# eth-cscs/COSTA

Hardware: AMD Instinct MI355X
Metric: GB/s device-resident tile pack+transpose+unpack (fp64), % HBM peak (higher is better)
Workload: dtype f64; 1 GPU; pxtran fp64 16384x16384, 256x256 blocks, op T, alpha=1 beta=0, 1x1 grid (BASELINE configs[1]); op=T, parallelism=1 rank(s), one per GPU, RCCL send/recv exchange, m=16384, n=16384, block=256, grid=1x1

## Files before the change

### costa_amd/__init__.py

```python
from __future__ import annotations

import ctypes as C
import os
import struct
from dataclasses import dataclass
from typing import Iterable, Sequence

import numpy as np

__all__ = [
    "CostaError", "lib", "FLOAT", "DOUBLE", "CFLOAT", "CDOUBLE", "INT32", "HALF", "BFLOAT16",
    "FP8_E4M3", "FP8_E5M2", "FP4_E2M1", "FP6_E2M3", "FP6_E3M2", "dtype_code", "element_code",
    "np_dtype", "Layout", "block_cyclic_layout", "custom_layout", "Comm", "transform",
    "transform_batch", "transform_async", "transform_batch_async", "synchronize", "transformer", "copy_and_transform", "execute_tiles", "execute_tiles_mixed",
    "convert_subtile", "TileOp", "TriOp", "TRI_OP_DTYPE", "transform_tri", "transform_tri_async",
    "execute_tiles_tri", "plan_export_tri", "tri_cut", "tri_subtile", "tri_phase_ms",
    "plan_export", "set_profiling", "get_stats", "release_caches", "TILE_OP_DTYPE",
    "ScaledOp", "SCALED_OP_DTYPE", "SCALED_F_ROWS", "transform_scaled", "execute_tiles_scaled",
    "plan_export_scaled", "scaled_subtile", "scaled_items", "mx_subtile", "block_subtile",
    "transform_amax", "layout_amax", "execute_tiles_amax", "amax_items",
    "MxScales", "MX_ROWS", "MX_COLS", "MX_FLOOR", "MX_CEIL", "mx_scales", "transform_mx",
    "execute_tiles_mx", "mx_items", "sr_bits", "mx_check_ops", "mx_check_scales",
    "BlockScales", "BLOCK_EXACT", "BLOCK_POW2", "block_scales", "transform_block_scaled",
    "execute_tiles_block_scaled", "block_items", "block_check_ops", "block_check_scales",
]

FLOAT, DOUBLE, CFLOAT, CDOUBLE, INT32 = 0, 1, 2, 3, 4
HALF, BFLOAT16 = 5, 6
_NP = {FLOAT: np.float32, DOUBLE: np.float64, CFLOAT: np.complex64,
       CDOUBLE: np.complex128, INT32: np.int32, HALF: np.float16, BFLOAT16: np.uint16}
_TORCH = {"torch.float32": FLOAT, "torch.float64": DOUBLE, "torch.complex64": CFLOAT,
          "torch.complex128": CDOUBLE, "torch.int32": INT32, "torch.float16": HALF,
# ... 252 lines not shown
        "costa_hip_mx_check_scales": (i, [C.POINTER(MxScales), i64, i64]),
        "costa_hip_plan_export_scaled": (i, [vp, vp, c, vp, vp, i, i, C.POINTER(ScaledPlanInfo), vp, vp,
                                             vp, vp, vp, vp, vp, vp]),
        "costa_hip_plan_export": (i, [i, C.POINTER(vp), C.POINTER(vp), C.c_char_p, vp, vp, i, i,
                                      C.POINTER(PlanInfo), vp, vp, vp, vp, vp, vp, vp, vp]),
        "costa_hip_set_profiling": (i, [i]),
        "costa_hip_get_stats": (i, [C.POINTER(FullStats), i]),
        "costa_hip_release_caches": (i, []),
        "costa_hip_set_host_staging": (i, [i]),
        "costa_hip_set_planner": (i, [i]),
        "costa_hip_plan_export_device": (i, [i, i, C.POINTER(vp), C.POINTER(vp), C.c_char_p, vp, vp,
                                             i, i, C.POINTER(PlanInfo), vp, vp, vp, vp, vp, vp, vp,
                                             vp]),
        "costa_hip_set_list_builder": (i, [i]),
        "costa_hip_work_export": (i, [i, vp, i64, i, i, vp, i64, vp, i64, C.POINTER(i64)]),
    }
    for name, (res, args) in sig.items():
        try:
            f = getattr(L, name)
        except AttributeError:
            if os.environ.get("COSTA_LIB"):
                continue
            raise
        f.restype = res
        f.argtypes = args
    _lib = L
    return L


def _check(rc: int):
# ... 843 lines not shown
    code = element_code(dtype)
    ops = np.ascontiguousarray(ops, dtype=TILE_OP_DTYPE)
    k = {"local": 0, "pack": 1, "unpack": 2}[kind]
    dev = -1 if device is None else int(device)
    meta = (C.c_int64 * 12)()
    L = lib()
    _check(L.costa_hip_work_export(code, ops.ctypes.data, ops.size, k, dev, None, 0, None, 0, meta))
    o = np.zeros(meta[8], TILE_OP_DTYPE)
    w = np.zeros(meta[9], np.uint64)
    _check(L.costa_hip_work_export(code, ops.ctypes.data, ops.size, k, dev, o.ctypes.data, o.size,
                                   w.ctypes.data, w.size, meta))
    m = dict(zip(_WORK_META, list(meta)))
    return WorkLists(o, w, m, bool(m["on_gpu"]))


def set_host_staging(mode: int):
    _check(lib().costa_hip_set_host_staging(int(mode)))


def rccl_version() -> int:
    v = C.c_int(0)
    _check(lib().costa_hip_rccl_version(C.byref(v)))
    return v.value
```

### costa_amd/csrc/capi.cpp

```cpp
#include "engine.hpp"

#include <hip/hip_runtime.h>

#include <costa/transform.hpp>

#include <algorithm>
#include <cctype>
#include <complex>
#include <cstring>
#include <new>

struct costa_layout_s {
    costa::engine::elayout e;
    std::vector<int> base_owners;
};
struct costa_comm_s {
    costa::engine::comm* c = nullptr;
};

namespace {
thread_local std::string g_last_error;

template <typename F>
int guarded(F&& f) {
// ... 984 lines not shown
        const bool on_gpu = costa::engine::work_export(
            costa_dtype_t(dtype), in, costa::engine::list_kind(kind), device, o, w, ws);
        const int64_t m[12] = {ws.n_large, ws.n_medium, ws.n_skew, ws.n_cblock, ws.cblock_lds, ws.cb_map,
                               ws.tiny_first, ws.n_tiny, int64_t(o.size()), int64_t(w.size()), on_gpu,
                               int64_t(ws.tr_shape) | int64_t(ws.sq) << 1 | int64_t(ws.full) << 2 |
                                   int64_t(ws.med_full) << 3 | int64_t(ws.med_sq) << 4 |
                                   int64_t(ws.skew_wide) << 5};
        std::memcpy(meta, m, sizeof(m));
        if (ordered && cap_ordered >= int64_t(o.size()) && !o.empty())
            std::memcpy(ordered, o.data(), o.size() * sizeof(o[0]));
        if (work && cap_work >= int64_t(w.size()) && !w.empty()) std::memcpy(work, w.data(), w.size() * sizeof(w[0]));
    };
    return device >= 0 ? gpu_guarded(body) : guarded(body);
}

int costa_hip_set_profiling(int on) {
    costa::engine::set_profiling(on != 0);
    return COSTA_OK;
}

int costa_hip_get_stats(costa_stats_t* out, int reset) {
    return guarded([&] {
        if (!out) throw costa::engine::error(COSTA_ERR_ARG, "null argument");
        costa::engine::resolve_pending();
        *out = costa::engine::stats();
        if (reset) costa::engine::stats() = costa_stats_t{};
    });
}

int costa_hip_set_host_staging(int mode) {
// ... 152 lines not shown
```

### costa_amd/csrc/engine.cpp

```cpp
#include <exception>
#include <thread>
#include "engine.hpp"
#include "strip_work.hpp"

#include <hip/hip_runtime.h>
#include <rccl/rccl.h>

#include <algorithm>
#include <numeric>
#include <chrono>
#include <cmath>
#include <cstdio>
#include <cstdlib>
#include <cstring>
#include <deque>
#include <list>
#include <map>
#include <mutex>
#include <unordered_map>

namespace costa {
namespace engine {

#define HIP_CHECK(x)                                                                   \
// ... 964 lines not shown
                out.push_back(head);
            }
            if (h < op.nf) {
                costa_tile_op_t body = part;
                body.src += uint64_t(h * E);
                body.dst += uint64_t(h * E);
                body.nf = int32_t(op.nf - h);
                body.flags = (op.flags & ~vec_bits) | vec_flags(body.src, body.lds, body.dst, body.ldd, E) | keep_vs;
                out.push_back(body);
            }
        }
    }
    return true;
}

work_split build_work(costa_dtype_t dtype, const std::vector<costa_tile_op_t>& ops_in,
                      std::vector<costa_tile_op_t>& ordered, std::vector<uint64_t>& work,
                      list_kind kind, device_section* dev, bool dst_order) {
    const bool pack_list = kind == list_pack, local = kind == list_local;
    static const int mis_env = [] {
        const char* s = tuning_env("COSTA_MISALIGNED_VEC");
        return s ? std::atoi(s) : -1;
    }();
    const int mis = mis_env >= 0 ? mis_env : dtype_size(dtype) == 4 ? 2 : 0;
    const wave_knobs& kn0 = knobs();
    static const bool trace = std::getenv("COSTA_PLAN_TRACE") != nullptr;
    const auto bw0 = std::chrono::steady_clock::now();
    double bw_t[4] = {0, 0, 0, 0};
    double sub_t[3] = {0, 0, 0};
    auto lap = [&](int k) {
        if (!trace) return;
        const double t = std::chrono::duration<double, std::milli>(std::chrono::steady_clock::now() - bw0).count();
        bw_t[k] = t;
// ... 136 lines not shown
        if (cls[li] == 1) --n_med;
        if (groups_on && op.ns <= op.ldd && op.ldd <= group_budget) {
            cls[li] = 2;
            continue;
        }
        cls[li] = 4;
    }
    mark(2);
    std::vector<uint32_t> shaped[3];
    std::vector<costa_tile_op_t> skew_ops;
    for (size_t li = 0; li < ops.size(); ++li) {
        const int c = cls[li] == 1 && n_med < kMinMediumOps ? 2 : cls[li];
        if (c < 2) shaped[c].push_back(uint32_t(li));
        else if (c == 2) wave_ops.push_back(&ops[li]);
        else if (c == 4) skew_ops.push_back(ops[li]);
    }
    merge_adjacent(skew_ops, E);
    for (size_t i = 0; i < skew_ops.size(); ++i) shaped[2].push_back(uint32_t(i));
    bool skew_wide = false;
    for (const auto& op : skew_ops)
        skew_wide = skew_wide || (E == 4 && (op.src % 16 != 0 || (uint64_t(op.lds) * uint64_t(E)) % 16 != 0));
    const int64_t skew_group = kn.skew_xcd >= 0 ? kn.skew_xcd : skew_wide ? kSkewWideGroup : 0;
    int64_t n_work[3] = {0, 0, 0};
    for (int c = 0; c < 3; ++c) {
        const int bf = c == 2 ? (skew_wide ? sh.bf_kw : sh.bf_k) : c ? (med_sq ? sh.bf_s : sh.bf_m) : sq ? sh.bf_q : sh.bf;
        const int bs = c == 2 ? (skew_wide ? sh.bs_kw : sh.bs_k) : c ? (med_sq ? sh.bs_s : sh.bs_m) : sq ? sh.bs_q : sh.bs;
        const std::vector<uint32_t>& sel = shaped[c];
        const std::vector<costa_tile_op_t>& src_ops = c == 2 ? skew_ops : ops;
        std::vector<uint32_t> sperm(sel.size());
        for (size_t i = 0; i < sel.size(); ++i) sperm[i] = uint32_t(i);
// ... 139 lines not shown
        std::sort(key.begin(), key.end());
        for (size_t i = 0; i < nw; ++i) perm[i] = key[i].second;
    } else {
        for (size_t i = 0; i < nw; ++i) perm[i] = uint32_t(i);
    }
    if (kn.xcd_bands && mode == 2 && top > 0 && nw > 1) xcd_bands(wave_ops, E, kn.xcd_bands, local, perm);
    lap(2);
    std::vector<wave_grid> grid(nw);
    std::vector<size_t> at_piece(nw + 1, 0);
    host_parallel(nw, [&](size_t b, size_t e) {
        for (size_t i = b; i < e; ++i) grid[i] = wave_pieces(*wave_ops[perm[i]], E, local);
    });
    for (size_t i = 0; i < nw; ++i)
        at_piece[i + 1] = at_piece[i] + size_t(grid[i].nfc * grid[i].nsc);
    work_split w;
    w.tr_shape = tr_shape;
    w.sq = sq;
    w.full = tr_shape && !sq && !shaped[0].empty();
    for (const uint32_t li : shaped[0]) {
        const costa_tile_op_t& op = ops[li];
        w.full = w.full && (op.flags & vec_both) == vec_both && op.nf % sh.bf == 0 && op.ns % sh.bs == 0;
    }
    w.med_sq = med_sq && !shaped[1].empty();
    w.med_full = !shaped[1].empty() && n_work[1] > 0 && !w.med_sq;
    for (const uint32_t li : shaped[1])
        w.med_full = w.med_full && ops[li].nf % sh.bf_m == 0 && ops[li].ns % sh.bs_m == 0;
    w.n_large = n_work[0];
    w.n_medium = n_work[1];
    w.n_skew = n_work[2];
    w.skew_wide = skew_wide && n_work[2] > 0;
// ... 167 lines not shown

void set_layout_hash(elayout& L) { layout_hashes(L, L.hash, L.hash2); }

namespace {

struct dev_list {
    dbuf ops, work;
    template <typename Op>
    const Op* list() const { return static_cast<const Op*>(ops.p); }
    const uint64_t* items() const { return static_cast<const uint64_t*>(work.p); }
};

struct phase_lists {
    dev_list tiles;
    work_split split;
    strip_list convert;
    bool transposes = false, reads_c = false;
    dev_list tri;
    strip_list tri_items;
    dev_list scaled;
    strip_list scaled_items;
    dbuf block_work;
    strip_list block_items;
    bool empty() const {
        return !split.n_items() && !convert.n_items && !tri_items.n_items && !scaled_items.n_items;
    }
};

struct cached_plan {
    std::unique_ptr<plan> p;
// ... 137 lines not shown
    sec.device = device;
    sec.stream = dc.main;
    sec.force = true;
    w = build_work(dtype, ops, ordered, work, kind, &sec);
    if (!sec.n_ordered) return false;
    std::vector<costa_tile_op_t> o(sec.n_ordered);
    std::vector<uint64_t> k(sec.n_work);
    HIP_CHECK(hipMemcpyAsync(o.data(), sec.d_ordered, o.size() * sizeof(o[0]), hipMemcpyDeviceToHost, dc.main));
    HIP_CHECK(hipMemcpyAsync(k.data(), sec.d_work, k.size() * sizeof(k[0]), hipMemcpyDeviceToHost, dc.main));
    HIP_CHECK(hipStreamSynchronize(dc.main));
    ordered.insert(ordered.begin() + std::ptrdiff_t(sec.at_ordered), o.begin(), o.end());
    work.insert(work.begin() + std::ptrdiff_t(sec.at_work), k.begin(), k.end());
    return true;
}

namespace {
std::unique_ptr<plan> plan_jobs(const std::vector<job>& jobs, comm* c, hipStream_t s) {
    const int lb = c->size == 1 && c->nccl ? loopback_exchange() : 0;
    const int mode = planner_mode();
    size_t blocks = 0;
    for (const job& j : jobs) blocks += j.A->blocks.size() + j.C->blocks.size();
    const size_t need = g_device_planner_warm ? kDevicePlanBlocks : kColdDevicePlanBlocks;
    if (!any_packed(jobs) && (mode == 2 || (mode == 1 && blocks >= need))) {
        if (auto p = make_plan_device(jobs, c->rank, c->size, lb, c->device, s)) {
            g_stats.device_plans++;
            g_device_planner_warm = true;
            return p;
        }
    }
    return make_plan(jobs, c->rank, c->size, lb);
// ... 38 lines not shown
        sec.stream = s;
    }
};

void build_phase(const plan& p, list_kind kind, bool masked, const std::vector<costa_tile_op_t>& tiles,
                 const std::vector<costa_tri_op_t>& tri, const std::vector<costa_scaled_op_t>& scaled,
                 host_lists& h) {
    phase_lists& ph = *h.into;
    const dtype_pair t = phase_dtypes(p, kind);
    ph.transposes = kind != list_pack && any_transpose(tiles);
    ph.reads_c = kind != list_pack && any_axpby(tiles);
    switch (phase_tiles(p, kind)) {
    case tiles_on::converting:
        ph.convert = build_convert_work(t.src, t.dst, tiles, 0, 0, h.tiles, h.tiles_work);
        break;
    case tiles_on::tile_kernel:
        ph.split = build_work(t.dst, tiles, h.tiles, h.tiles_work, kind, kind == list_pack ? nullptr : &h.sec,
                              kind == list_local && masked);
        break;
    case tiles_on::none:
        break;
    }
    if (!tri.empty()) ph.tri_items = build_tri_work(t.dst, tri, 0, 0, h.tri, h.tri_work);
    if (scaled.empty()) return;
    static const bool local_by_dst = [] {
        const char* e = tuning_env("COSTA_SCALED_ORDER");
        return !e || std::atoi(e) != 0;
    }();
    const bool by_dst = kind == list_local && local_by_dst;
    ph.scaled_items = build_scaled_work(t.src, t.dst, scaled, 0, 0, h.scaled, h.scaled_work, by_dst);
    if (block_pair(p.src_dtype, p.dtype) && dtype_is_fp8(p.dtype)) {
        std::vector<costa_scaled_op_t> same;
        ph.block_items = build_block_work(t.src, t.dst, scaled, 0, 0, same, h.block_work, by_dst);
    }
}

void upload_phase(const host_lists& h, hipStream_t s) {
    phase_lists& ph = *h.into;
    upload_list(ph.tiles.ops, h.tiles, h.sec.d_ordered, h.sec.at_ordered, h.sec.n_ordered, s);
    upload_list(ph.tiles.work, h.tiles_work, h.sec.d_work, h.sec.at_work, h.sec.n_work, s);
    if (ph.tri_items.n_items) {
        ph.tri.ops.upload(h.tri, s);
        ph.tri.work.upload(h.tri_work, s);
    }
    if (ph.scaled_items.n_items) {
        ph.scaled.ops.upload(h.scaled, s);
        ph.scaled.work.upload(h.scaled_work, s);
    }
    if (ph.block_items.n_items) ph.block_work.upload(h.block_work, s);
}

template <typename Op>
std::vector<std::vector<Op>> by_round(const std::vector<Op>& ops, const std::vector<int>& round, int R) {
    std::vector<std::vector<Op>> out(static_cast<size_t>(R));
    for (size_t i = 0; i < ops.size(); ++i) out[size_t(round[i])].push_back(ops[i]);
    return out;
}

std::vector<host_lists> build_lists(cached_plan& cp, comm* c, hipStream_t s, bool masked) {
    const plan& p = *cp.p;
    if (p.packed() && (!p.local_ops.empty() || !p.unpack_ops.empty()))
        throw error(COSTA_ERR_INTERNAL, "costa: an FP4 / FP6 plan with ordinary LOCAL / UNPACK ops");
    const int R = c->exchanges() ? exchange_rounds() : 1;
    std::vector<int> pr, ur, tr, sr;
// ... 197 lines not shown
    if (masked || device_only(jobs)) {
        costa_dtype_t a, b;
        check_jobs(jobs, c->size, a, b);
    }
    auto cp = std::make_unique<cached_plan>();
    cp->device = c->device;
    staging st;
    if (stage_host_layouts(jobs, c, dc, masked, *cp, st)) return cp;
    const double t_resid = now_ms() - t0;
    cp->p = plan_jobs(st.jobs, c, dc.main);
    const double t_plan = now_ms() - t0 - t_resid;
    g_stats.plan_ms += t_plan;
    if (cp->staged) staged_copies(*cp, st, masked);
    const std::vector<host_lists> lists = build_lists(*cp, c, dc.main, masked);
    const double t_work = now_ms() - t0 - t_resid - t_plan;
    for (const host_lists& h : lists) upload_phase(h, dc.main);
    HIP_CHECK(hipStreamSynchronize(dc.main));
    if (trace)
        std::fprintf(stderr,
                     "[costa plan] %zu local / %zu pack / %zu unpack ops: residency %.2f ms, "
                     "planning %.2f, work lists %.2f, upload %.2f, total %.2f\n",
                     cp->p->local_ops.size(), cp->p->pack_ops.size(), cp->p->unpack_ops.size(), t_resid, t_plan,
                     t_work, now_ms() - t0 - t_resid - t_plan - t_work, now_ms() - t0);
    return cp;
}

cached_plan* get_plan(const std::vector<job>& jobs, comm* c, device_ctx& dc) {
    std::vector<uint64_t> key = plan_key(jobs, c);
    hasher h;
    for (uint64_t w : key) h.mix(w);
    for (auto it = g_plans.begin(); it != g_plans.end(); ++it) {
        if (it->h == h.h && it->key == key) {
// ... 28 lines not shown

void release_caches() {
    std::lock_guard<std::recursive_mutex> lk(g_mutex);
    g_plans.clear();
    release_host_rings();
    ctx_map().clear();
}

namespace {
enum phase { PH_LOCAL, PH_PACK, PH_EXCHANGE, PH_UNPACK, PH_H2D, PH_D2H, PH_TRI_LOCAL, PH_TRI_UNPACK };
double g_tri_ms = 0;
int64_t g_scaled_items = 0;
int64_t g_amax_items = 0;
int64_t g_mx_items = 0;
int64_t g_blk_items = 0;

struct phase_timer {
    device_ctx& dc;
    bool on;
    int ph = 0;
    hipEvent_t a = nullptr;
    hipStream_t s = nullptr;
    phase_timer(device_ctx& d, bool prof) : dc(d), on(prof) {}
    void start(int p, hipStream_t st) {
        if (!on) return;
        ph = p;
        s = st;
        a = dc.take_event();
        HIP_CHECK(hipEventRecord(a, s));
    }
// ... 35 lines not shown
        hipEvent_t e;
        HIP_CHECK(hipEventCreate(&e));
        return e;
    }
    hipEvent_t e = free_events.back();
    free_events.pop_back();
    return e;
}

void resolve_pending() {
    std::lock_guard<std::recursive_mutex> lk(g_mutex);
    for (auto& kv : ctx_map()) {
        HIP_CHECK(hipSetDevice(kv.first));
        kv.second->resolve();
    }
}

double tri_phase_ms(bool reset) {
    resolve_pending();
    std::lock_guard<std::recursive_mutex> lk(g_mutex);
    const double v = g_tri_ms;
    if (reset) g_tri_ms = 0;
    return v;
}

void synchronize(comm* c) {
    std::lock_guard<std::recursive_mutex> lk(g_mutex);
    if (!c) throw error(COSTA_ERR_ARG, "costa: null communicator");
    device_ctx& dc = ctx(c->device);
    HIP_CHECK(hipStreamSynchronize(dc.main));
// ... 183 lines not shown
    const int id = kind == list_local ? PH_LOCAL : kind == list_pack ? PH_PACK : PH_UNPACK;
    const void* scal = cp.d_scal.p;
    auto launch = [&](int phase, auto&& run) {
        if (after) HIP_CHECK(hipStreamWaitEvent(s, after, 0));
        tm.start(phase, s);
        run();
        tm.stop();
    };
    if (ph.convert.n_items)
        launch(id, [&] {
            launch_convert(t.src, t.dst, ph.tiles.list<costa_tile_op_t>(), ph.tiles.items(), ph.convert, src_base,
                           dst_base, scal, s);
        });
    if (ph.split.n_items())
        launch(id, [&] {
            launch_tiles(t.dst,
                         make_launch(ph.split, ph.tiles.ops.p, ph.tiles.work.p, src_base, dst_base, scal,
                                     ph.transposes, ph.reads_c),
                         s);
        });
    if (ph.tri_items.n_items)
        launch(kind == list_local ? PH_TRI_LOCAL : PH_TRI_UNPACK, [&] {
            launch_tri(t.dst, ph.tri.list<costa_tri_op_t>(), ph.tri.items(), ph.tri_items, src_base, dst_base, scal, s);
        });
    if (ph.scaled_items.n_items)
        launch(id, [&] {
            const costa_scaled_op_t* ops = ph.scaled.list<costa_scaled_op_t>();
            switch (sv.scheme) {
            case scale_scheme::block:
                launch_block(t.src, t.dst, ops,
                             sv.quantises() ? static_cast<const uint64_t*>(ph.block_work.p) : ph.scaled.items(),
                             sv.quantises() ? ph.block_items : ph.scaled_items, src_base, dst_base, scal,
                             sv.blk.a_scales, sv.blk.c_scales, sv.blk.pow2, s);
                break;
// ... 731 lines not shown
```

### costa_amd/csrc/engine.hpp

```cpp
#pragma once

#include <costa/layout.hpp>
#include <costa_hip.h>

#include <array>
#include <cstdint>
#include <functional>
#include <memory>
#include <string>
#include <vector>

#include "tile_op.hpp"

namespace costa {
namespace engine {

size_t dtype_size(costa_dtype_t t);
esize elem_size(costa_dtype_t t);
bool dtype_is_complex(costa_dtype_t t);
bool dtype_is_half(costa_dtype_t t);
costa_dtype_t compute_dtype(costa_dtype_t src, costa_dtype_t dst);
bool half_pair(costa_dtype_t src, costa_dtype_t dst);
bool dtype_is_fp8(costa_dtype_t t);
bool fp8_pair(costa_dtype_t src, costa_dtype_t dst);
// ... 289 lines not shown
    const char* src_base;
    char* dst_base;
    const void* scalars;
    bool any_transpose;
    bool any_axpby;
    bool tr_shape;
    bool sq;
    bool full;
    bool med_full;
    bool med_sq;
    bool skew_wide = false;
};
bool any_transpose(const std::vector<costa_tile_op_t>& ops);
bool any_axpby(const std::vector<costa_tile_op_t>& ops);
void launch_tiles(costa_dtype_t dtype, const launch_args& a, void* stream );
bool pieces_in_group_launch(int64_t n_cblock, int64_t n_tiny);
constexpr int64_t kPanelBytes = int64_t(128) << 10;
constexpr int kCblockThreads = 256;
constexpr int kCblockChunks = 4;
inline int64_t cblock_max_elems(int64_t E) { return int64_t(kCblockThreads) * kCblockChunks * (16 / E); }
constexpr int64_t kCblockXcdChunk = 16;
constexpr int64_t cblock_xcd_order(int64_t b, int64_t nb, int64_t ch = kCblockXcdChunk) {
    return b / (8 * ch) * (8 * ch) + 8 * ch <= nb ? b / (8 * ch) * (8 * ch) + (b % 8) * ch + (b / 8) % ch : b;
}
constexpr int64_t xcd_slice_order(int64_t b, int64_t nb) {
    return (b % 8) < nb % 8 ? (b % 8) * (nb / 8 + 1) + b / 8
                            : (nb % 8) * (nb / 8 + 1) + ((b % 8) - nb % 8) * (nb / 8) + b / 8;
}
enum cblock_map { cb_round_robin = 0, cb_xcd_chunks = 1, cb_xcd_bands = 2 };
struct shape_dims {
// ... 17 lines not shown
    bool skew_wide = false;
    int64_t n_items() const { return n_large + n_medium + n_skew + n_cblock + n_tiny; }
};
enum list_kind { list_local, list_pack, list_unpack };
struct device_section {
    int device = -1;
    void* stream = nullptr;
    bool force = false;
    std::shared_ptr<void> mem;
    costa_tile_op_t* d_ordered = nullptr;
    uint64_t* d_work = nullptr;
    size_t at_ordered = 0, n_ordered = 0, at_work = 0, n_work = 0;
};
work_split build_work(costa_dtype_t dtype, const std::vector<costa_tile_op_t>& ops,
                      std::vector<costa_tile_op_t>& ordered, std::vector<uint64_t>& work,
                      list_kind kind = list_local, device_section* dev = nullptr, bool dst_order = false);
constexpr size_t kDeviceGroupsMin = 16384;
int list_builder_mode();
void set_list_builder_mode(int mode);
int64_t cblock_groups_device(int64_t E, int64_t budget, uint32_t vec_bits, int bands_env,
                             const std::vector<costa_tile_op_t>& ops, const std::vector<uint32_t>& wave,
                             size_t base_at, device_section& sec, std::vector<char>& taken,
                             int64_t& lds, int& map);
bool work_export(costa_dtype_t dtype, const std::vector<costa_tile_op_t>& ops, list_kind kind,
                 int device, std::vector<costa_tile_op_t>& ordered, std::vector<uint64_t>& work,
                 work_split& w);
launch_args make_launch(const work_split& w, const void* d_ordered, const void* d_work,
                        const char* src_base, char* dst_base, const void* d_scalars, bool transpose,
                        bool axpby);

struct host_pipeline;
// ... 31 lines not shown
```

### costa_amd/csrc/tile_kernels.hip

```cpp
#include <hip/hip_runtime.h>

#include <algorithm>
#include <cstdlib>
#include <type_traits>

#include "engine.hpp"
#include "tile_device.hpp"

#pragma clang fp contract(off)

namespace costa {
namespace engine {
namespace {

template <typename T, int V, int EPS>
__device__ __forceinline__ vec<T> shifted_chunk(const vec<T>& below, const vec<T>& o) {
    vec<T> c;
#pragma unroll
    for (int e = 0; e < V; ++e)
        c.e[e] = e < EPS ? below.e[V - EPS + e < V ? V - EPS + e : V - 1] : o.e[e >= EPS ? e - EPS : 0];
    return c;
}
template <typename T, typename S, bool NT>
__device__ __forceinline__ void store_shifted(T* d, const vec<T>& o, int n, int lane) {
// ... 305 lines not shown
    const int f0 = int(sub % uint32_t(nbf)) * S::BF;
    const int s0 = int(sub / uint32_t(nbf)) * S::BS;
    const int tf = min(S::BF, op.nf - f0);
    const int ts = min(S::BS, op.ns - s0);
    const uint32_t slot = op.flags >> COSTA_SLOT_SHIFT;
    const T alpha = scalars[2 * slot];
    const T beta = scalars[2 * slot + 1];
    const uint32_t vec_both = COSTA_TILE_VEC_SRC | COSTA_TILE_VEC_DST;
    constexpr bool NT = true;
    if (tf == S::BF && ts == S::BS && (op.flags & vec_both) == vec_both)
        run_tile<T, S, true, NT>(op, f0, s0, tf, ts, src_base, dst_base, alpha, beta, tile);
    else
        run_tile<T, S, false, NT>(op, f0, s0, tf, ts, src_base, dst_base, alpha, beta, tile);
}

template <typename T, bool WIDE = false>
struct skew_shape {
    static constexpr int NT = 512;
    static constexpr int BF = sizeof(T) == 4 ? (WIDE ? 64 : 32) : 64;
    static constexpr int BS = sizeof(T) == 4 ? (WIDE ? 256 : 512) : 128;
    static constexpr int E = int(sizeof(T)), G = 64 / E, RS = BS + G, P = BF + 1;
    static constexpr int V = 16 / E, LPC = BF / V, CPP = NT / LPC, PL = (RS + CPP - 1) / CPP;
    static constexpr int NW = NT / 64;
    static constexpr size_t lds_bytes = size_t(RS) * P * sizeof(T);
    static_assert(BS * E % 64 == 0, "sub-tile rows: whole granules");
};

template <typename T, bool WIDE>
__global__ __launch_bounds__(512) void skew_kernel(const costa_tile_op_t* __restrict__ ops,
                                                   const uint64_t* __restrict__ work,
// ... 527 lines not shown
    d->bf_s = tr ? shapes<T>::small32_tr::BF : 0;
    d->bs_s = tr ? shapes<T>::small32_tr::BS : 0;
    constexpr bool skew = std::is_same<T, float>::value || std::is_same<T, double>::value ||
                          std::is_same<T, int>::value;
    d->bf_k = tr && skew ? skew_shape<T>::BF : 0;
    d->bs_k = tr && skew ? skew_shape<T>::BS : 0;
    d->bf_kw = tr && skew ? skew_shape<T, true>::BF : 0;
    d->bs_kw = tr && skew ? skew_shape<T, true>::BS : 0;
}

template <typename T, typename S>
void set_lds_limit() {
    (void)hipFuncSetAttribute(reinterpret_cast<const void*>(&tile_kernel<T, S>),
                              hipFuncAttributeMaxDynamicSharedMemorySize, int(S::lds_bytes));
}
template <typename T>
void set_lds_limits() {
    if constexpr (std::is_same<T, float>::value || std::is_same<T, double>::value ||
                  std::is_same<T, int>::value)
    {
        (void)hipFuncSetAttribute(reinterpret_cast<const void*>(&skew_kernel<T, false>),
                                  hipFuncAttributeMaxDynamicSharedMemorySize,
                                  int(skew_shape<T, false>::lds_bytes));
        (void)hipFuncSetAttribute(reinterpret_cast<const void*>(&skew_kernel<T, true>),
                                  hipFuncAttributeMaxDynamicSharedMemorySize,
                                  int(skew_shape<T, true>::lds_bytes));
    }
    if constexpr (!is_cpx<T>::value)
        for (void* f : {reinterpret_cast<void*>(&cblock_kernel<T, true, true>),
                        reinterpret_cast<void*>(&cblock_kernel<T, true, false>),
                        reinterpret_cast<void*>(&cblock_kernel<T, false, true>),
                        reinterpret_cast<void*>(&cblock_kernel<T, false, false>)})
            (void)hipFuncSetAttribute(f, hipFuncAttributeMaxDynamicSharedMemorySize,
                                      int((cblock_max_elems(int64_t(sizeof(T))) + 4096) * int64_t(sizeof(T))));
    set_lds_limit<T, typename shapes<T>::large>();
    set_lds_limit<T, typename shapes<T>::large_tr>();
    set_lds_limit<T, typename shapes<T>::medium_tr>();
    set_lds_limit<T, typename shapes<T>::small_tr>();
    set_lds_limit<T, typename shapes<T>::large_tr_full>();
    set_lds_limit<T, typename shapes<T>::medium_tr_full>();
    set_lds_limit<T, typename shapes<T>::small32_tr>();
}

}

bool pieces_in_group_launch(int64_t n_cblock, int64_t n_tiny) {
    static const bool on = [] {
        const char* v = tuning_env("COSTA_FUSE_PIECES");
        return !v || std::atoi(v) != 0;
    }();
    return on && n_cblock > 0 && n_tiny > 0 && n_cblock + n_tiny / (CB_NT / 64) + 1 < (int64_t(1) << 30);
}

void tile_shapes(costa_dtype_t dtype, bool transposing_list, shape_dims* d) {
    const bool t = transposing_list;
    switch (dtype) {
    case COSTA_FLOAT: shape_of<float>(t, d); return;
    case COSTA_DOUBLE: shape_of<double>(t, d); return;
    case COSTA_CFLOAT: shape_of<cpx<float>>(t, d); return;
    case COSTA_CDOUBLE: shape_of<cpx<double>>(t, d); return;
    case COSTA_INT32: shape_of<int>(t, d); return;
    default: break;
    }
    throw error(COSTA_ERR_ARG, "unknown dtype");
}

void launch_tiles(costa_dtype_t dtype, const launch_args& a, void* stream) {
    if (a.n_large + a.n_medium + a.n_skew + a.n_cblock + a.n_tiny <= 0) return;
    static bool once = [] {
        set_lds_limits<float>();
        set_lds_limits<double>();
        set_lds_limits<cpx<float>>();
        set_lds_limits<cpx<double>>();
        set_lds_limits<int>();
        return true;
    }();
    (void)once;
    hipStream_t s = static_cast<hipStream_t>(stream);
    switch (dtype) {
    case COSTA_FLOAT: launch_t<float>(a, s); break;
    case COSTA_DOUBLE: launch_t<double>(a, s); break;
    case COSTA_CFLOAT: launch_t<cpx<float>>(a, s); break;
    case COSTA_CDOUBLE: launch_t<cpx<double>>(a, s); break;
    case COSTA_INT32: launch_t<int>(a, s); break;
    default: throw error(COSTA_ERR_ARG, std::string("costa: no same-type tile kernel for ") + dtype_name(dtype));
    }
    hipError_t e = hipGetLastError();
    if (e != hipSuccess)
        throw error(COSTA_ERR_HIP, std::string("tile kernel launch failed: ") + hipGetErrorString(e));
}

}
}
```

### costa_amd/csrc/tile_op.hpp

```cpp
#pragma once

#include <cstdint>

#include "costa_hip.h"

#if defined(__HIPCC__)
#define COSTA_HD __host__ __device__
#else
#define COSTA_HD
#endif

namespace costa {
namespace engine {

struct esize {
    uint64_t qb;
    COSTA_HD constexpr esize(uint64_t bytes) : qb(4 * bytes) {}
    COSTA_HD static constexpr esize packed(unsigned bits) {
        esize e(0);
        e.qb = bits / 2;
        return e;
    }
    COSTA_HD constexpr uint64_t bytes(uint64_t n) const { return n * qb / 4; }
};
// ... 75 lines not shown
COSTA_HD inline costa_tile_op_t& tile_of(costa_tile_op_t& o) { return o; }
COSTA_HD inline costa_tile_op_t& tile_of(costa_tri_op_t& o) { return o.op; }
COSTA_HD inline costa_tile_op_t& tile_of(costa_scaled_op_t& o) { return o.op; }

COSTA_HD inline int64_t tri_kept(const costa_tri_op_t& t) {
    const bool le = t.op.flags & COSTA_TRI_LE;
    int64_t n = 0;
    for (int64_t s = 0; s < t.op.ns; ++s) {
        const int64_t x = s - t.diag;
        const int64_t c = le ? int64_t(t.op.nf) - x : x + 1;
        n += c < 0 ? 0 : c > t.op.nf ? t.op.nf : c;
    }
    return n;
}

COSTA_HD inline int64_t op_alg_bytes(const costa_tile_op_t& op, esize elem) {
    const uint32_t k = (op.flags & COSTA_SCALE_MASK) >> COSTA_SCALE_SHIFT;
    const int64_t n = int64_t(op.nf) * op.ns;
    return int64_t(elem.bytes(uint64_t(n))) * (1 + (k != COSTA_SCALE_ZERO) + (k == COSTA_SCALE_AXPBY));
}
COSTA_HD inline int64_t op_alg_bytes(const costa_tile_op_t& op, esize src_elem, esize dst_elem) {
    const uint32_t k = (op.flags & COSTA_SCALE_MASK) >> COSTA_SCALE_SHIFT;
    const int64_t n = int64_t(op.nf) * op.ns;
    return int64_t(src_elem.bytes(uint64_t(n))) * (k != COSTA_SCALE_ZERO) +
           int64_t(dst_elem.bytes(uint64_t(n))) * (1 + (k == COSTA_SCALE_AXPBY));
}

COSTA_HD inline int64_t op_alg_bytes(const costa_tri_op_t& t, esize elem) {
    const uint32_t k = (t.op.flags & COSTA_SCALE_MASK) >> COSTA_SCALE_SHIFT;
    return int64_t(elem.bytes(uint64_t(tri_kept(t)))) * (1 + (k != COSTA_SCALE_ZERO) + (k == COSTA_SCALE_AXPBY));
// ... 5 lines not shown
```

### include/costa_hip.h

```cpp
#ifndef COSTA_HIP_H
#define COSTA_HIP_H

#include <stddef.h>
#include <stdint.h>

#ifdef __cplusplus
extern "C" {
#endif

#define COSTA_OK 0
#define COSTA_ERR_ARG 1
#define COSTA_ERR_HIP 2
#define COSTA_ERR_NCCL 3
#define COSTA_ERR_INTERNAL 4

typedef enum {
    COSTA_FLOAT = 0,
    COSTA_DOUBLE = 1,
    COSTA_CFLOAT = 2,
    COSTA_CDOUBLE = 3,
    COSTA_INT32 = 4,
    COSTA_HALF = 5,
    COSTA_BFLOAT16 = 6,
    COSTA_FP8_E4M3 = 7,
// ... 291 lines not shown

int costa_hip_set_host_staging(int mode);

int costa_hip_set_planner(int mode);
int costa_hip_plan_export_device(int device, int n, const costa_layout_t* A, const costa_layout_t* C,
                                 const char* trans, const void* alpha, const void* beta, int rank,
                                 int nranks, costa_plan_info_t* info, costa_tile_op_t* local_ops,
                                 costa_tile_op_t* pack_ops, costa_tile_op_t* unpack_ops,
                                 int64_t* send_counts, int64_t* send_displs, int64_t* recv_counts,
                                 int64_t* recv_displs, void* scalars);

int costa_hip_set_list_builder(int mode);
int costa_hip_work_export(int dtype, const costa_tile_op_t* ops, int64_t n_ops, int kind, int device,
                          costa_tile_op_t* ordered, int64_t cap_ordered, uint64_t* work,
                          int64_t cap_work, int64_t* meta);

#ifdef __cplusplus
}
#endif
#endif
```

Measured before the change: 6194 GB/s.

## Replace uploaded tile work lists with an implicit lattice descriptor for regular local ops

Detects when local tile ops form a regular 2D lattice with uniform strides and shapes, and encodes them as a compact grid descriptor passed by value to a new grid kernel. The kernel recomputes op and sub-tile positions with fast-division arithmetic instead of reading per-item work and op lists from device memory. This also skips list uploads and the extra stream synchronisation when nothing needs uploading. The cost is extra index arithmetic per block plus more detection code paths that must match the existing ordering (panel and by-destination) exactly.

```diff
diff --git a/costa_amd/__init__.py b/costa_amd/__init__.py
--- a/costa_amd/__init__.py
+++ b/costa_amd/__init__.py
@@ -15,7 +15,7 @@
     "transform_batch", "transform_async", "transform_batch_async", "synchronize", "transformer", "copy_and_transform", "execute_tiles", "execute_tiles_mixed",
     "convert_subtile", "TileOp", "TriOp", "TRI_OP_DTYPE", "transform_tri", "transform_tri_async",
     "execute_tiles_tri", "plan_export_tri", "tri_cut", "tri_subtile", "tri_phase_ms",
-    "plan_export", "set_profiling", "get_stats", "release_caches", "TILE_OP_DTYPE",
+    "plan_export", "grid_export", "grid_launches", "set_profiling", "get_stats", "release_caches", "TILE_OP_DTYPE",
     "ScaledOp", "SCALED_OP_DTYPE", "SCALED_F_ROWS", "transform_scaled", "execute_tiles_scaled",
     "plan_export_scaled", "scaled_subtile", "scaled_items", "mx_subtile", "block_subtile",
     "transform_amax", "layout_amax", "execute_tiles_amax", "amax_items",
@@ -298,6 +298,8 @@
                                              vp]),
         "costa_hip_set_list_builder": (i, [i]),
         "costa_hip_work_export": (i, [i, vp, i64, i, i, vp, i64, vp, i64, C.POINTER(i64)]),
+        "costa_hip_grid_export": (i, [i, vp, i64, i, C.POINTER(i64), vp, i64, vp, i64]),
+        "costa_hip_grid_launches": (i, [C.POINTER(i64), i]),
     }
     for name, (res, args) in sig.items():
         try:
@@ -1171,6 +1173,39 @@
     return WorkLists(o, w, m, bool(m["on_gpu"]))
 
 
+@dataclass
+class GridLists:
+    is_grid: bool
+    desc: dict
+    ordered: np.ndarray
+    work: np.ndarray
+
+
+_GRID_DESC = ("is_grid", "n_ordered", "n_work", "ni", "nj", "sa", "sb", "da", "db", "bf", "bs", "nbf", "nbs",
+              "by_dst", "n_row", "n_col", "mul_row", "mul_col", "panel_rows", "panel_subs", "flags")
+
+
+def grid_export(dtype, ops: np.ndarray, kind: str = "local") -> GridLists:
+    code = element_code(dtype)
+    ops = np.ascontiguousarray(ops, dtype=TILE_OP_DTYPE)
+    k = {"local": 0, "pack": 1, "unpack": 2}[kind]
+    desc = (C.c_int64 * 24)()
+    L = lib()
+    _check(L.costa_hip_grid_export(code, ops.ctypes.data, ops.size, k, desc, None, 0, None, 0))
+    o = np.zeros(desc[1], TILE_OP_DTYPE)
+    w = np.zeros(desc[2], np.uint64)
+    if desc[0]:
+        _check(L.costa_hip_grid_export(code, ops.ctypes.data, ops.size, k, desc, o.ctypes.data, o.size,
+                                       w.ctypes.data, w.size))
+    return GridLists(bool(desc[0]), dict(zip(_GRID_DESC, list(desc))), o, w)
+
+
+def grid_launches(reset: bool = False) -> int:
+    v = C.c_int64(0)
+    _check(lib().costa_hip_grid_launches(C.byref(v), int(reset)))
+    return v.value
+
+
 def set_host_staging(mode: int):
     _check(lib().costa_hip_set_host_staging(int(mode)))
 
diff --git a/costa_amd/csrc/capi.cpp b/costa_amd/csrc/capi.cpp
--- a/costa_amd/csrc/capi.cpp
+++ b/costa_amd/csrc/capi.cpp
@@ -1022,6 +1022,39 @@
     return device >= 0 ? gpu_guarded(body) : guarded(body);
 }
 
+int costa_hip_grid_export(int dtype, const costa_tile_op_t* ops, int64_t n_ops, int kind, int64_t* desc,
+                          costa_tile_op_t* ordered, int64_t cap_ordered, uint64_t* work, int64_t cap_work) {
+    return guarded([&] {
+        if (!desc || (n_ops > 0 && !ops) || n_ops < 0) throw costa::engine::error(COSTA_ERR_ARG, "null argument");
+        if (dtype < COSTA_FLOAT || dtype > COSTA_INT32) throw costa::engine::error(COSTA_ERR_ARG, "bad dtype");
+        if (kind < 0 || kind > 2) throw costa::engine::error(COSTA_ERR_ARG, "kind must be 0, 1 or 2");
+        std::vector<costa_tile_op_t> in(ops, ops + n_ops);
+        costa::engine::grid_desc g;
+        costa::engine::work_split ws;
+        const bool is_grid = costa::engine::grid_export(costa_dtype_t(dtype), in, costa::engine::list_kind(kind), g, ws);
+        const int64_t n_ordered = is_grid ? int64_t(g.ni) * g.nj : 0, n_work = is_grid ? ws.n_large : 0;
+        const int64_t d[24] = {is_grid, n_ordered, n_work, g.ni, g.nj, g.sa, g.sb, g.da, g.db, g.bf, g.bs, g.nbf,
+                               g.nbs, g.by_dst, g.n_row, g.n_col, g.mul_row, g.mul_col, g.panel_rows, g.panel_subs,
+                               int64_t(ws.tr_shape) | int64_t(ws.sq) << 1 | int64_t(ws.full) << 2, 0, 0, 0};
+        std::memcpy(desc, d, sizeof(d));
+        if (!is_grid) return;
+        if (ordered && cap_ordered >= n_ordered)
+            for (int64_t i = 0; i < n_ordered; ++i) ordered[i] = costa::engine::grid_op(g, uint32_t(i));
+        if (work && cap_work >= n_work)
+            for (int64_t k = 0; k < n_work; ++k) {
+                const costa::engine::grid_pos at = costa::engine::grid_item(g, uint32_t(k));
+                work[k] = uint64_t(at.op) << 32 | at.sub;
+            }
+    });
+}
+
+int costa_hip_grid_launches(int64_t* n, int reset) {
+    return guarded([&] {
+        if (!n) throw costa::engine::error(COSTA_ERR_ARG, "null argument");
+        *n = costa::engine::grid_launches(reset != 0);
+    });
+}
+
 int costa_hip_set_profiling(int on) {
     costa::engine::set_profiling(on != 0);
     return COSTA_OK;
diff --git a/costa_amd/csrc/engine.cpp b/costa_amd/csrc/engine.cpp
--- a/costa_amd/csrc/engine.cpp
+++ b/costa_amd/csrc/engine.cpp
@@ -1002,9 +1002,109 @@
     return true;
 }
 
+namespace {
+bool grid_enabled() {
+    static const bool on = [] {
+        const char* s = tuning_env("COSTA_GRID");
+        return !s || std::atoi(s) != 0;
+    }();
+    return on;
+}
+
+bool detect_grid(costa_dtype_t dtype, const std::vector<costa_tile_op_t>& ops_in, int64_t E, int bf, int bs,
+                 bool sq, const wave_knobs& kn, grid_desc& g) {
+    const size_t n = ops_in.size();
+    if (n == 0 || n > 0xFFFFFFFFull) return false;
+    bool hints = true, ascending = true;
+    for (size_t k = 0; k < n; ++k) {
+        hints = hints && ops_in[k].order != 0;
+        ascending = ascending && (k == 0 || ops_in[k - 1].order <= ops_in[k].order);
+    }
+    std::vector<costa_tile_op_t> by_hint;
+    if (kn.large_sort >= 1 && hints && !ascending) {
+        by_hint = ops_in;
+        std::stable_sort(by_hint.begin(), by_hint.end(),
+                         [](const costa_tile_op_t& x, const costa_tile_op_t& y) { return x.order < y.order; });
+    }
+    const std::vector<costa_tile_op_t>& ops = by_hint.empty() ? ops_in : by_hint;
+    const costa_tile_op_t& o = ops[0];
+    const uint32_t vec_both = COSTA_TILE_VEC_SRC | COSTA_TILE_VEC_DST;
+    if ((o.flags & vec_both) != vec_both || o.nf % bf != 0 || o.ns % bs != 0) return false;
+    if ((int64_t(o.lds) * E) % 16 != 0 || (int64_t(o.ldd) * E) % 16 != 0) return false;
+    const int64_t nbf = o.nf / bf, nbs = o.ns / bs;
+    if (int64_t(n) * nbf * nbs > (int64_t(1) << 30)) return false;
+    const int64_t sb = n > 1 ? int64_t(ops[1].src - o.src) : 0, db = n > 1 ? int64_t(ops[1].dst - o.dst) : 0;
+    size_t nj = n;
+    for (size_t k = 2; k < n; ++k)
+        if (int64_t(ops[k].src - ops[k - 1].src) != sb || int64_t(ops[k].dst - ops[k - 1].dst) != db) {
+            nj = k;
+            break;
+        }
+    if (n % nj != 0) return false;
+    const size_t ni = n / nj;
+    const int64_t sa = ni > 1 ? int64_t(ops[nj].src - o.src) : 0, da = ni > 1 ? int64_t(ops[nj].dst - o.dst) : 0;
+    for (size_t k = 0; k < n; ++k) {
+        const costa_tile_op_t& x = ops[k];
+        const int64_t i = int64_t(k / nj), j = int64_t(k % nj);
+        if (x.nf != o.nf || x.ns != o.ns || x.lds != o.lds || x.ldd != o.ldd || x.flags != o.flags) return false;
+        if (x.src != o.src + uint64_t(i * sa + j * sb) || x.dst != o.dst + uint64_t(i * da + j * db)) return false;
+        if (x.src % 16 != 0 || x.dst % 16 != 0) return false;
+    }
+    g = grid_desc{};
+    g.src0 = o.src;
+    g.dst0 = o.dst;
+    g.sa = sa, g.sb = sb, g.da = da, g.db = db;
+    g.ni = int32_t(ni), g.nj = int32_t(nj);
+    g.nf = o.nf, g.ns = o.ns, g.lds = o.lds, g.ldd = o.ldd;
+    g.flags = o.flags;
+    g.bf = bf, g.bs = bs;
+    g.nbf = int32_t(nbf), g.nbs = int32_t(nbs);
+    const bool tr = o.flags & COSTA_TILE_TRANSPOSE;
+    const bool by_address = kn.large_sort == 2 || (kn.large_sort == 3 && (E == 4 || E == 8 || (E == 16 && sq)) && tr);
+    if (!by_address || grid_items(g) < 2) {
+        grid_finish(g);
+        return true;
+    }
+    if (!tr) return false;
+    const int64_t col = int64_t(o.ldd) * E;
+    int64_t step_row = 0, step_col = 0;
+    g.n_row = g.n_col = 1;
+    for (int d = 0; d < 2; ++d) {
+        const int64_t cnt = d ? int64_t(nj) : int64_t(ni), step = d ? db : da, mul = d ? 1 : int64_t(nj);
+        if (cnt == 1) continue;
+        if (step <= 0) return false;
+        if (step % col == 0) {
+            if (g.n_col > 1 || step / col < o.nf) return false;
+            g.n_col = int32_t(cnt), g.mul_col = int32_t(mul), step_col = step / col;
+        } else {
+            if (g.n_row > 1 || step >= col || step % E != 0 || step / E < o.ns) return false;
+            g.n_row = int32_t(cnt), g.mul_row = int32_t(mul), step_row = step / E;
+        }
+    }
+    if (int64_t(g.n_row - 1) * step_row + o.ns > o.ldd) return false;
+    g.by_dst = 1;
+    int64_t panel = kn.panel_rows;
+    if (panel == 0) panel = col > kPanelBytes && dtype != COSTA_CFLOAT ? kPanelBytes / E : -1;
+    if (panel >= (int64_t(1) << 24)) panel = -1;
+    if (panel > 0) {
+        const uint64_t ld = uint64_t(o.ldd);
+        const uint64_t last = uint64_t(g.n_col - 1) * uint64_t(step_col) * ld + uint64_t(o.nf - bf) * ld +
+                              uint64_t(g.n_row - 1) * uint64_t(step_row) + uint64_t(o.ns - bs);
+        const bool fits = last / ld < (uint64_t(1) << 24) && ld / uint64_t(panel) < (uint64_t(1) << 16);
+        if (fits) {
+            if ((g.n_row > 1 && step_row != o.ns) || panel % bs != 0) return false;
+            g.panel_rows = int32_t(panel);
+            g.panel_subs = int32_t(panel / bs);
+        }
+    }
+    grid_finish(g);
+    return true;
+}
+}
+
 work_split build_work(costa_dtype_t dtype, const std::vector<costa_tile_op_t>& ops_in,
                       std::vector<costa_tile_op_t>& ordered, std::vector<uint64_t>& work,
-                      list_kind kind, device_section* dev, bool dst_order) {
+                      list_kind kind, device_section* dev, bool dst_order, grid_desc* lattice) {
     const bool pack_list = kind == list_pack, local = kind == list_local;
     static const int mis_env = [] {
         const char* s = tuning_env("COSTA_MISALIGNED_VEC");
@@ -1171,6 +1271,25 @@
         if (c < 2) shaped[c].push_back(uint32_t(li));
         else if (c == 2) wave_ops.push_back(&ops[li]);
         else if (c == 4) skew_ops.push_back(ops[li]);
+    }
+    if (lattice && !dst_order && grid_enabled() && !ops.empty() && shaped[0].size() == ops.size() &&
+        detect_grid(dtype, ops, E, sq ? sh.bf_q : sh.bf, sq ? sh.bs_q : sh.bs, sq, kn, *lattice)) {
+        work_split w;
+        std::memset(static_cast<void*>(&w), 0, sizeof(w));
+        w.tr_shape = tr_shape;
+        w.sq = sq;
+        w.full = tr_shape && !sq;
+        w.n_large = int64_t(grid_items(*lattice));
+        w.tiny_first = int64_t(ops.size());
+        if (trace) {
+            lap(0);
+            std::fprintf(stderr,
+                         "[costa build_work] %zu ops (local list): a %d x %d lattice of %d x %d sub-tiles, %.2f ms "
+                         "(merge %.2f, flags + granules %.2f, classify %.2f)\n",
+                         ops_in.size(), lattice->ni, lattice->nj, lattice->nbf, lattice->nbs, bw_t[0], sub_t[0],
+                         sub_t[1] - sub_t[0], sub_t[2] - sub_t[1]);
+        }
+        return w;
     }
     merge_adjacent(skew_ops, E);
     for (size_t i = 0; i < skew_ops.size(); ++i) shaped[2].push_back(uint32_t(i));
@@ -1340,6 +1459,7 @@
     for (size_t i = 0; i < nw; ++i)
         at_piece[i + 1] = at_piece[i] + size_t(grid[i].nfc * grid[i].nsc);
     work_split w;
+    std::memset(static_cast<void*>(&w), 0, sizeof(w));
     w.tr_shape = tr_shape;
     w.sq = sq;
     w.full = tr_shape && !sq && !shaped[0].empty();
@@ -1537,6 +1657,8 @@
 struct phase_lists {
     dev_list tiles;
     work_split split;
+    bool is_grid = false;
+    grid_desc grid{};
     strip_list convert;
     bool transposes = false, reads_c = false;
     dev_list tri;
@@ -1704,6 +1826,16 @@
     return true;
 }
 
+bool grid_export(costa_dtype_t dtype, const std::vector<costa_tile_op_t>& ops, list_kind kind, grid_desc& g,
+                 work_split& w) {
+    std::lock_guard<std::recursive_mutex> lk(g_mutex);
+    std::vector<costa_tile_op_t> ordered;
+    std::vector<uint64_t> work;
+    g = grid_desc{};
+    w = build_work(dtype, ops, ordered, work, kind, nullptr, false, kind == list_local ? &g : nullptr);
+    return w.n_large > 0 && ordered.empty() && work.empty();
+}
+
 namespace {
 std::unique_ptr<plan> plan_jobs(const std::vector<job>& jobs, comm* c, hipStream_t s) {
     const int lb = c->size == 1 && c->nccl ? loopback_exchange() : 0;
@@ -1772,10 +1904,14 @@
     case tiles_on::converting:
         ph.convert = build_convert_work(t.src, t.dst, tiles, 0, 0, h.tiles, h.tiles_work);
         break;
-    case tiles_on::tile_kernel:
+    case tiles_on::tile_kernel: {
+        const bool try_grid = kind == list_local && !masked && !p.converting() && !p.scaled && tri.empty() &&
+                              scaled.empty();
         ph.split = build_work(t.dst, tiles, h.tiles, h.tiles_work, kind, kind == list_pack ? nullptr : &h.sec,
-                              kind == list_local && masked);
+                              kind == list_local && masked, try_grid ? &ph.grid : nullptr);
+        ph.is_grid = try_grid && ph.split.n_large > 0 && h.tiles.empty() && h.tiles_work.empty();
         break;
+    }
     case tiles_on::none:
         break;
     }
@@ -1793,8 +1929,11 @@
     }
 }
 
-void upload_phase(const host_lists& h, hipStream_t s) {
+bool upload_phase(const host_lists& h, hipStream_t s) {
     phase_lists& ph = *h.into;
+    if (h.tiles.empty() && h.tiles_work.empty() && !h.sec.n_ordered && !h.sec.n_work && !h.sec.mem &&
+        h.tri.empty() && h.tri_work.empty() && h.scaled.empty() && h.scaled_work.empty() && h.block_work.empty())
+        return false;
     upload_list(ph.tiles.ops, h.tiles, h.sec.d_ordered, h.sec.at_ordered, h.sec.n_ordered, s);
     upload_list(ph.tiles.work, h.tiles_work, h.sec.d_work, h.sec.at_work, h.sec.n_work, s);
     if (ph.tri_items.n_items) {
@@ -1806,6 +1945,7 @@
         ph.scaled.work.upload(h.scaled_work, s);
     }
     if (ph.block_items.n_items) ph.block_work.upload(h.block_work, s);
+    return true;
 }
 
 template <typename Op>
@@ -2033,8 +2173,9 @@
     if (cp->staged) staged_copies(*cp, st, masked);
     const std::vector<host_lists> lists = build_lists(*cp, c, dc.main, masked);
     const double t_work = now_ms() - t0 - t_resid - t_plan;
-    for (const host_lists& h : lists) upload_phase(h, dc.main);
-    HIP_CHECK(hipStreamSynchronize(dc.main));
+    bool uploaded = false;
+    for (const host_lists& h : lists) uploaded = upload_phase(h, dc.main) || uploaded;
+    if (uploaded) HIP_CHECK(hipStreamSynchronize(dc.main));
     if (trace)
         std::fprintf(stderr,
                      "[costa plan] %zu local / %zu pack / %zu unpack ops: residency %.2f ms, "
@@ -2093,6 +2234,7 @@
 int64_t g_amax_items = 0;
 int64_t g_mx_items = 0;
 int64_t g_blk_items = 0;
+int64_t g_grid_launches = 0;
 
 struct phase_timer {
     device_ctx& dc;
@@ -2158,6 +2300,13 @@
         HIP_CHECK(hipSetDevice(kv.first));
         kv.second->resolve();
     }
+}
+
+int64_t grid_launches(bool reset) {
+    std::lock_guard<std::recursive_mutex> lk(g_mutex);
+    const int64_t v = g_grid_launches;
+    if (reset) g_grid_launches = 0;
+    return v;
 }
 
 double tri_phase_ms(bool reset) {
@@ -2371,10 +2520,14 @@
         });
     if (ph.split.n_items())
         launch(id, [&] {
-            launch_tiles(t.dst,
-                         make_launch(ph.split, ph.tiles.ops.p, ph.tiles.work.p, src_base, dst_base, scal,
-                                     ph.transposes, ph.reads_c),
-                         s);
+            const launch_args a = make_launch(ph.split, ph.tiles.ops.p, ph.tiles.work.p, src_base, dst_base, scal,
+                                              ph.transposes, ph.reads_c);
+            if (ph.is_grid) {
+                launch_grid(t.dst, ph.grid, a, s);
+                ++g_grid_launches;
+            } else {
+                launch_tiles(t.dst, a, s);
+            }
         });
     if (ph.tri_items.n_items)
         launch(kind == list_local ? PH_TRI_LOCAL : PH_TRI_UNPACK, [&] {
diff --git a/costa_amd/csrc/engine.hpp b/costa_amd/csrc/engine.hpp
--- a/costa_amd/csrc/engine.hpp
+++ b/costa_amd/csrc/engine.hpp
@@ -327,6 +327,7 @@
 bool any_transpose(const std::vector<costa_tile_op_t>& ops);
 bool any_axpby(const std::vector<costa_tile_op_t>& ops);
 void launch_tiles(costa_dtype_t dtype, const launch_args& a, void* stream );
+void launch_grid(costa_dtype_t dtype, const grid_desc& g, const launch_args& a, void* stream );
 bool pieces_in_group_launch(int64_t n_cblock, int64_t n_tiny);
 constexpr int64_t kPanelBytes = int64_t(128) << 10;
 constexpr int kCblockThreads = 256;
@@ -374,7 +375,11 @@
 };
 work_split build_work(costa_dtype_t dtype, const std::vector<costa_tile_op_t>& ops,
                       std::vector<costa_tile_op_t>& ordered, std::vector<uint64_t>& work,
-                      list_kind kind = list_local, device_section* dev = nullptr, bool dst_order = false);
+                      list_kind kind = list_local, device_section* dev = nullptr, bool dst_order = false,
+                      grid_desc* grid = nullptr);
+bool grid_export(costa_dtype_t dtype, const std::vector<costa_tile_op_t>& ops, list_kind kind, grid_desc& g,
+                 work_split& w);
+int64_t grid_launches(bool reset);
 constexpr size_t kDeviceGroupsMin = 16384;
 int list_builder_mode();
 void set_list_builder_mode(int mode);
diff --git a/costa_amd/csrc/tile_kernels.hip b/costa_amd/csrc/tile_kernels.hip
--- a/costa_amd/csrc/tile_kernels.hip
+++ b/costa_amd/csrc/tile_kernels.hip
@@ -343,6 +343,22 @@
         run_tile<T, S, false, NT>(op, f0, s0, tf, ts, src_base, dst_base, alpha, beta, tile);
 }
 
+template <typename T, typename S>
+__global__ __launch_bounds__(S::NT) void tile_grid_kernel(const grid_desc g, const char* src_base,
+                                                          char* dst_base, const T* __restrict__ scalars) {
+    extern __shared__ __attribute__((aligned(16))) unsigned char smem[];
+    T* tile = reinterpret_cast<T*>(smem);
+    const grid_pos at = grid_item(g, blockIdx.x);
+    const costa_tile_op_t op = grid_op(g, at.op);
+    const uint32_t si = at.sub / g.q_nbf;
+    const int f0 = int(at.sub - si * uint32_t(g.nbf)) * S::BF;
+    const int s0 = int(si) * S::BS;
+    const uint32_t slot = g.flags >> COSTA_SLOT_SHIFT;
+    const T alpha = scalars[2 * slot];
+    const T beta = scalars[2 * slot + 1];
+    run_tile<T, S, true, true>(op, f0, s0, S::BF, S::BS, src_base, dst_base, alpha, beta, tile);
+}
+
 template <typename T, bool WIDE = false>
 struct skew_shape {
     static constexpr int NT = 512;
@@ -900,6 +916,11 @@
     (void)hipFuncSetAttribute(reinterpret_cast<const void*>(&tile_kernel<T, S>),
                               hipFuncAttributeMaxDynamicSharedMemorySize, int(S::lds_bytes));
 }
+template <typename T, typename S>
+void set_grid_lds_limit() {
+    (void)hipFuncSetAttribute(reinterpret_cast<const void*>(&tile_grid_kernel<T, S>),
+                              hipFuncAttributeMaxDynamicSharedMemorySize, int(S::lds_bytes));
+}
 template <typename T>
 void set_lds_limits() {
     if constexpr (std::is_same<T, float>::value || std::is_same<T, double>::value ||
@@ -926,6 +947,41 @@
     set_lds_limit<T, typename shapes<T>::large_tr_full>();
     set_lds_limit<T, typename shapes<T>::medium_tr_full>();
     set_lds_limit<T, typename shapes<T>::small32_tr>();
+    set_grid_lds_limit<T, typename shapes<T>::large>();
+    set_grid_lds_limit<T, typename shapes<T>::small_tr>();
+    set_grid_lds_limit<T, typename shapes<T>::large_tr_full>();
+}
+
+void set_all_lds_limits() {
+    static bool once = [] {
+        set_lds_limits<float>();
+        set_lds_limits<double>();
+        set_lds_limits<cpx<float>>();
+        set_lds_limits<cpx<double>>();
+        set_lds_limits<int>();
+        return true;
+    }();
+    (void)once;
+}
+
+template <typename T, typename S>
+void launch_grid_shape(const grid_desc& g, const launch_args& a, hipStream_t stream) {
+    if (g.bf != S::BF || g.bs != S::BS) throw error(COSTA_ERR_INTERNAL, "costa: lattice list cut with another shape");
+    const size_t lds = a.any_transpose ? S::lds_bytes : 0;
+    hipLaunchKernelGGL((tile_grid_kernel<T, S>), dim3(unsigned(a.n_large)), dim3(S::NT), lds, stream, g,
+                       a.src_base, a.dst_base, static_cast<const T*>(a.scalars));
+}
+template <typename T>
+void launch_grid_t(const grid_desc& g, const launch_args& a, hipStream_t stream) {
+    if (a.sq) {
+        if (!shapes<T>::has_small || !a.tr_shape) throw error(COSTA_ERR_INTERNAL, "costa: square shape");
+        launch_grid_shape<T, typename shapes<T>::small_tr>(g, a, stream);
+    } else if (a.tr_shape) {
+        if (!a.full) throw error(COSTA_ERR_INTERNAL, "costa: lattice list of partial sub-tiles");
+        launch_grid_shape<T, typename shapes<T>::large_tr_full>(g, a, stream);
+    } else {
+        launch_grid_shape<T, typename shapes<T>::large>(g, a, stream);
+    }
 }
 
 }
@@ -953,15 +1009,7 @@
 
 void launch_tiles(costa_dtype_t dtype, const launch_args& a, void* stream) {
     if (a.n_large + a.n_medium + a.n_skew + a.n_cblock + a.n_tiny <= 0) return;
-    static bool once = [] {
-        set_lds_limits<float>();
-        set_lds_limits<double>();
-        set_lds_limits<cpx<float>>();
-        set_lds_limits<cpx<double>>();
-        set_lds_limits<int>();
-        return true;
-    }();
-    (void)once;
+    set_all_lds_limits();
     hipStream_t s = static_cast<hipStream_t>(stream);
     switch (dtype) {
     case COSTA_FLOAT: launch_t<float>(a, s); break;
@@ -976,5 +1024,25 @@
         throw error(COSTA_ERR_HIP, std::string("tile kernel launch failed: ") + hipGetErrorString(e));
 }
 
-}
-}
+void launch_grid(costa_dtype_t dtype, const grid_desc& g, const launch_args& a, void* stream) {
+    if (a.n_large <= 0) return;
+    if (uint64_t(a.n_large) != grid_items(g) || a.n_large > (int64_t(1) << 30) ||
+        a.n_medium + a.n_skew + a.n_cblock + a.n_tiny != 0)
+        throw error(COSTA_ERR_INTERNAL, "costa: lattice list with other work items");
+    set_all_lds_limits();
+    hipStream_t s = static_cast<hipStream_t>(stream);
+    switch (dtype) {
+    case COSTA_FLOAT: launch_grid_t<float>(g, a, s); break;
+    case COSTA_DOUBLE: launch_grid_t<double>(g, a, s); break;
+    case COSTA_CFLOAT: launch_grid_t<cpx<float>>(g, a, s); break;
+    case COSTA_CDOUBLE: launch_grid_t<cpx<double>>(g, a, s); break;
+    case COSTA_INT32: launch_grid_t<int>(g, a, s); break;
+    default: throw error(COSTA_ERR_ARG, std::string("costa: no same-type tile kernel for ") + dtype_name(dtype));
+    }
+    hipError_t e = hipGetLastError();
+    if (e != hipSuccess)
+        throw error(COSTA_ERR_HIP, std::string("tile kernel launch failed: ") + hipGetErrorString(e));
+}
+
+}
+}
diff --git a/costa_amd/csrc/tile_op.hpp b/costa_amd/csrc/tile_op.hpp
--- a/costa_amd/csrc/tile_op.hpp
+++ b/costa_amd/csrc/tile_op.hpp
@@ -113,6 +113,91 @@
     return n;
 }
 
+struct fast_div {
+    uint32_t d, m, s;
+};
+COSTA_HD inline fast_div fast_div_of(uint32_t d) {
+    fast_div x{d ? d : 1u, 0u, 0u};
+    if (x.d > 1) {
+        while ((uint64_t(2) << x.s) < x.d) ++x.s;
+        x.m = uint32_t(((uint64_t(1) << (32 + x.s)) + x.d - 1) / x.d);
+    }
+    return x;
+}
+COSTA_HD inline uint32_t operator/(uint32_t n, const fast_div& x) {
+    return x.d == 1 ? n : uint32_t((uint64_t(n) * x.m) >> 32) >> x.s;
+}
+
+struct grid_desc {
+    uint64_t src0, dst0;
+    int64_t sa, sb, da, db;
+    int32_t ni, nj;
+    int32_t nf, ns, lds, ldd;
+    uint32_t flags;
+    int32_t bf, bs;
+    int32_t nbf, nbs;
+    uint32_t by_dst;
+    int32_t n_row, n_col, mul_row, mul_col;
+    int32_t panel_rows;
+    int32_t panel_subs;
+    fast_div q_nj, q_nbf, q_nbs, q_per, q_rows, q_panel, q_ps, q_last;
+};
+
+COSTA_HD inline void grid_finish(grid_desc& g) {
+    const uint32_t nbf = uint32_t(g.nbf), nbs = uint32_t(g.nbs);
+    const uint32_t NR = uint32_t(g.n_row) * nbs, NC = uint32_t(g.n_col) * nbf, ps = uint32_t(g.panel_subs);
+    g.q_nj = fast_div_of(uint32_t(g.nj));
+    g.q_nbf = fast_div_of(nbf);
+    g.q_nbs = fast_div_of(nbs);
+    g.q_per = fast_div_of(nbf * nbs);
+    g.q_rows = fast_div_of(NR);
+    g.q_panel = fast_div_of(ps * NC);
+    g.q_ps = fast_div_of(ps);
+    g.q_last = fast_div_of(ps ? NR % ps : 0u);
+}
+
+COSTA_HD inline uint64_t grid_items(const grid_desc& g) {
+    return uint64_t(g.ni) * uint64_t(g.nj) * uint64_t(g.nbf) * uint64_t(g.nbs);
+}
+
+COSTA_HD inline costa_tile_op_t grid_op(const grid_desc& g, uint32_t idx) {
+    const uint32_t i = idx / g.q_nj, j = idx - i * uint32_t(g.nj);
+    costa_tile_op_t op{};
+    op.src = g.src0 + uint64_t(int64_t(i) * g.sa + int64_t(j) * g.sb);
+    op.dst = g.dst0 + uint64_t(int64_t(i) * g.da + int64_t(j) * g.db);
+    op.nf = g.nf;
+    op.ns = g.ns;
+    op.lds = g.lds;
+    op.ldd = g.ldd;
+    op.flags = g.flags;
+    return op;
+}
+
+struct grid_pos {
+    uint32_t op, sub;
+};
+COSTA_HD inline grid_pos grid_item(const grid_desc& g, uint32_t k) {
+    const uint32_t nbf = uint32_t(g.nbf), nbs = uint32_t(g.nbs);
+    if (!g.by_dst) {
+        const uint32_t op = k / g.q_per;
+        return {op, k - op * (nbf * nbs)};
+    }
+    const uint32_t NR = uint32_t(g.n_row) * nbs, NC = uint32_t(g.n_col) * nbf;
+    uint32_t r, c;
+    if (g.panel_subs > 0) {
+        const uint32_t ps = uint32_t(g.panel_subs);
+        const uint32_t p = k / g.q_panel, rem = k - p * (ps * NC);
+        const bool whole = NR - p * ps >= ps;
+        c = whole ? rem / g.q_ps : rem / g.q_last;
+        r = p * ps + (rem - c * (whole ? ps : NR - p * ps));
+    } else {
+        c = k / g.q_rows;
+        r = k - c * NR;
+    }
+    const uint32_t ir = r / g.q_nbs, si = r - ir * nbs, ic = c / g.q_nbf, fi = c - ic * nbf;
+    return {ir * uint32_t(g.mul_row) + ic * uint32_t(g.mul_col), si * nbf + fi};
+}
+
 COSTA_HD inline int64_t op_alg_bytes(const costa_tile_op_t& op, esize elem) {
     const uint32_t k = (op.flags & COSTA_SCALE_MASK) >> COSTA_SCALE_SHIFT;
     const int64_t n = int64_t(op.nf) * op.ns;
diff --git a/include/costa_hip.h b/include/costa_hip.h
--- a/include/costa_hip.h
+++ b/include/costa_hip.h
@@ -329,6 +329,9 @@
 int costa_hip_work_export(int dtype, const costa_tile_op_t* ops, int64_t n_ops, int kind, int device,
                           costa_tile_op_t* ordered, int64_t cap_ordered, uint64_t* work,
                           int64_t cap_work, int64_t* meta);
+int costa_hip_grid_export(int dtype, const costa_tile_op_t* ops, int64_t n_ops, int kind, int64_t* desc,
+                          costa_tile_op_t* ordered, int64_t cap_ordered, uint64_t* work, int64_t cap_work);
+int costa_hip_grid_launches(int64_t* n, int reset);
 
 #ifdef __cplusplus
 }
```

After: 6210 GB/s (median of 6 runs). About the same (+0.3%).
